# equinor/gordo-components

Hardware: NVIDIA B200
Metric: anomaly windows/sec (64-tag feedforward_hourglass AE, 1k machines x 10k rows per GPU, fused predict+score) (higher is better)
Workload: dtype tf32x3

## Files before the change

gordo_components_b200/csrc/ffae_infer_tc.cu:

```cuda
#include <cuda.h>
#include <atomic>
#include <cstdlib>
#include <cuda_bf16.h>
#include <cuda_fp16.h>
#include "gb_common.cuh"

namespace {

constexpr int TILE = 128;
#ifndef GB_TC_NSLOT
#define GB_TC_NSLOT 2
#endif
#ifndef GB_TC_YPREF
#define GB_TC_YPREF 2
#endif
#ifndef GB_TC_YPREF_LAYER
#define GB_TC_YPREF_LAYER 4
#endif
#ifndef GB_TC_STATIC
#define GB_TC_STATIC 1
#endif
constexpr int NSLOT = GB_TC_NSLOT;
static_assert(NSLOT == 2 || NSLOT == 3, "two or three tile slots");
#ifndef GB_TC_DEDICATED
#define GB_TC_DEDICATED 0
#endif
constexpr int MAIN_WARPS = 8, LAYER_GROUPS = GB_TC_DEDICATED ? NSLOT : 1, OUT0 = MAIN_WARPS * LAYER_GROUPS, OUT_WARPS = 8, EPI_WARPS = OUT0 + OUT_WARPS;
constexpr int NTHREADS = 32 * (EPI_WARPS + NSLOT);
constexpr int MAXL = 8;
constexpr int BOX_BYTES = TILE * 128;
constexpr int OBOX_BYTES = 32 * 128;
constexpr int W = 64;

constexpr uint32_t COL_D = 0, COL_A1 = 64, COL_A2 = 96, COL_ALB = GB_TC_DEDICATED ? 128 : 64, COL_ABF = GB_TC_DEDICATED ? 160 : 96,
                   SLOT_COLS = GB_TC_DEDICATED ? 192 : 128, COL_DX = NSLOT * SLOT_COLS, TMEM_COLS = 512;
static_assert(COL_DX + (GB_TC_DEDICATED ? NSLOT : NSLOT - 1) * 64 <= TMEM_COLS, "tile slots + spare accumulators exceed the 512 TMEM columns");

struct TcArgs {
  int T;
  int n_layers, last_layer;
  int K[MAXL], N[MAXL], Np[MAXL], n8[MAXL], k8[MAXL], k16[MAXL], act[MAXL];
  int whi_ofs[MAXL], wlo_ofs[MAXL], bias_ofs[MAXL];
  int whb_ofs;
  int pofs[MAXL];
  int w_bytes;
  int param_bytes, bulk_params;
  int vec_ofs, xbox_ofs, stage_ofs, pair_ofs, bar_ofs;
  int n_jobs, tiles_per_job, flags;
  long pstride;
  const float* params;
  const gb_job* jobs;
  const float *y, *scale, *feat_thr, *agg_thr;
  float *o_model, *o_ts, *o_tu, *o_conf, *o_tots, *o_totu, *o_totconf;
  unsigned int* work_ctr;
  long long* trace;
  int trace_cap, trace_from, trace_head;
};

enum { FLAG_NO_STORES = 2 };
constexpr int DEFAULT_NE = 0;

constexpr int TRACE_SLOTS = NSLOT == 2 ? 256 : 32;
__device__ __forceinline__ void trace_ev(const TcArgs& a, unsigned long long* ring, int& cnt, int code, int tile, int layer, int slot) {
  if (a.trace == nullptr || blockIdx.x != 0 || cnt >= TRACE_SLOTS || (tile < a.trace_from && tile >= a.trace_head)) return;
  ring[cnt++] = ((unsigned long long)clock64() << 24) | ((unsigned long long)(tile & 0xfff) << 12) | ((layer & 0xf) << 8) | ((slot & 0xf) << 4) | (code & 0xf);
}

__device__ __forceinline__ uint32_t smem_u32(const void* p) { return (uint32_t)__cvta_generic_to_shared(p); }

__device__ __forceinline__ void mbar_init(uint32_t bar, uint32_t count) {
  asm volatile("mbarrier.init.shared::cta.b64 [%0], %1;" ::"r"(bar), "r"(count));
}
__device__ __forceinline__ void mbar_arrive(uint32_t bar) {
  asm volatile("mbarrier.arrive.shared::cta.b64 _, [%0];" ::"r"(bar) : "memory");
}
__device__ __forceinline__ void mbar_expect_tx(uint32_t bar, uint32_t bytes) {
  asm volatile("mbarrier.arrive.expect_tx.shared::cta.b64 _, [%0], %1;" ::"r"(bar), "r"(bytes) : "memory");
}
__device__ __forceinline__ void mbar_wait(uint32_t bar, uint32_t parity) {
  asm volatile(
      "{\n\t"
      ".reg .pred p;\n\t"
      "WAIT_%=:\n\t"
      "mbarrier.try_wait.parity.shared::cta.b64 p, [%0], %1, %2;\n\t"
      "@p bra DONE_%=;\n\t"
      "bra WAIT_%=;\n\t"
      "DONE_%=:\n\t"
      "}" ::"r"(bar), "r"(parity), "r"(0x989680u)
      : "memory");
}
__device__ __forceinline__ void named_bar_sync(int id, int count) { asm volatile("bar.sync %0, %1;" ::"r"(id), "r"(count) : "memory"); }
__device__ __forceinline__ void fence_proxy_async() { asm volatile("fence.proxy.async.shared::cta;" ::: "memory"); }
__device__ __forceinline__ void tc_fence_before() { asm volatile("tcgen05.fence::before_thread_sync;" ::: "memory"); }
__device__ __forceinline__ void tc_fence_after() { asm volatile("tcgen05.fence::after_thread_sync;" ::: "memory"); }

__device__ __forceinline__ void tma_load_2d(uint32_t dst, const CUtensorMap* map, int c0, int c1, uint32_t bar) {
  asm volatile("cp.async.bulk.tensor.2d.shared::cluster.global.mbarrier::complete_tx::bytes [%0], [%1, {%2, %3}], [%4];" ::"r"(dst),
               "l"(map), "r"(c0), "r"(c1), "r"(bar)
               : "memory");
}

__device__ __forceinline__ void mma_bf16_ts(uint32_t d, uint32_t a, uint64_t bdesc, uint32_t idesc, uint32_t accumulate) {
  asm volatile(
      "{\n\t"
      ".reg .pred p;\n\t"
      "setp.ne.b32 p, %4, 0;\n\t"
      "tcgen05.mma.cta_group::1.kind::f16 [%0], [%1], %2, %3, p;\n\t"
      "}" ::"r"(d), "r"(a), "l"(bdesc), "r"(idesc), "r"(accumulate)
      : "memory");
}
__device__ __forceinline__ void mma_tf32_ss(uint32_t d, uint64_t adesc, uint64_t bdesc, uint32_t idesc, uint32_t accumulate) {
  asm volatile(
      "{\n\t"
      ".reg .pred p;\n\t"
      "setp.ne.b32 p, %4, 0;\n\t"
// ... 147 lines not shown
      v[i + j] = (NE > 0 && ((i + j) % (NE > 0 ? NE : 1)) == 0) ? tanh_from_scaled_fma(t[j]) : tanh_from_scaled(t[j]);
  }
  store_a_fp16<NC>(slot_lane, col0, v);
}
template <int C1, int C2, int NE>
__device__ __forceinline__ void hidden_epilogue_pair(uint32_t slot_lane, int c0, const float* bias_all) {
  hidden_epilogue<C1, NE>(slot_lane, c0, bias_all + c0);
  if (C2 > 0) hidden_epilogue<(C2 > 0 ? C2 : 4), NE>(slot_lane, c0 + C1, bias_all + c0 + C1);
}

__device__ __forceinline__ bool elect_one() {
  uint32_t pred;
  asm volatile("{\n\t.reg .pred P;\n\telect.sync _|P, 0xffffffff;\n\tselp.b32 %0, 1, 0, P;\n\t}" : "=r"(pred));
  return pred != 0;
}

template <int V> struct IC {};
constexpr int HG_L = 7;
constexpr int HG_DIMS[HG_L + 1] = {64, 53, 43, 32, 32, 43, 53, 64};
constexpr int hg_ru(int v, int m) { return (v + m - 1) / m * m; }
template <int l> struct HGL {
  static constexpr int K = HG_DIMS[l], N = HG_DIMS[l + 1];
  static constexpr int Np = hg_ru(N, 16), n8 = hg_ru(N, 8), k8 = hg_ru(K, 8) / 8, k16 = hg_ru(K, 16) / 16;
  static constexpr int whi_bytes = l == 0 ? k8 * 8 * Np * 4 : k16 * 16 * Np * 2, wlo_bytes = k16 * 16 * Np * 2, whb_bytes = l == 0 ? k16 * 16 * Np * 2 : 0;
  static constexpr int whi_ofs = HGL<l - 1>::end_ofs, wlo_ofs = whi_ofs + whi_bytes, whb_ofs = wlo_ofs + wlo_bytes, end_ofs = whb_ofs + whb_bytes;
};
template <> struct HGL<-1> { static constexpr int end_ofs = 0; };
template <int l> constexpr int HG_BIAS_OFS = HGL<HG_L - 1>::end_ofs + 64 * 4 * l;

struct LayerP { int K, N, Np, n8, k8, k16, whi_ofs, wlo_ofs, bias_ofs; };
template <int V> __device__ __forceinline__ LayerP layer_of(const TcArgs&, IC<V>) {
  return LayerP{HGL<V>::K, HGL<V>::N, HGL<V>::Np, HGL<V>::n8, HGL<V>::k8, HGL<V>::k16, HGL<V>::whi_ofs, HGL<V>::wlo_ofs, HG_BIAS_OFS<V>};
}
__device__ __forceinline__ LayerP layer_of(const TcArgs& a, int l) {
  return LayerP{a.K[l], a.N[l], a.Np[l], a.n8[l], a.k8[l], a.k16[l], a.whi_ofs[l], a.wlo_ofs[l], a.bias_ofs[l]};
}
template <int V> __device__ __forceinline__ constexpr int layer_index(IC<V>) { return V; }
__device__ __forceinline__ int layer_index(int l) { return l; }
template <bool STATIC, bool HIDDEN_ONLY, class F>
__device__ __forceinline__ void for_layers(int n, F&& f) {
  if constexpr (STATIC) {
    f(IC<0>{}); f(IC<1>{}); f(IC<2>{}); f(IC<3>{}); f(IC<4>{}); f(IC<5>{});
    if constexpr (!HIDDEN_ONLY) f(IC<6>{});
  } else {
    for (int l = 0; l < n; ++l) f(l);
  }
}

template <int NE, bool FULL, bool STATIC>
__global__ void __launch_bounds__(NTHREADS, 1)
ffae_tc_kernel(const __grid_constant__ TcArgs a, const __grid_constant__ CUtensorMap map_x) {
  extern __shared__ __align__(1024) uint8_t smem[];
  __shared__ uint32_t s_tmem_base;
  __shared__ unsigned long long s_trace[4][TRACE_SLOTS];
  int trace_cnt = 0;

  const int tid = threadIdx.x, lane = tid & 31;
  if (a.trace != nullptr && tid == 0) {
    unsigned long long ns;
    asm volatile("mov.u64 %0, %globaltimer;" : "=l"(ns));
    a.trace[8 + 4 * TRACE_SLOTS + 2 * blockIdx.x] = (long long)ns;
    if (blockIdx.x == 0) {
      a.trace[4 + 4 * TRACE_SLOTS + 0] = clock64();
      a.trace[4 + 4 * TRACE_SLOTS + 2] = (long long)ns;
    }
  }
  const int warp = __shfl_sync(0xffffffffu, tid >> 5, 0);
  const bool is_ctrl = warp >= EPI_WARPS, is_out = !is_ctrl && warp >= OUT0;
  unsigned long long* ring = s_trace[is_ctrl ? (warp == EPI_WARPS ? 1 : 0) : (is_out ? (warp == EPI_WARPS - 1 ? 2 : 3) : 0)];
  const int q = warp & 3, h = (warp >> 2) & 1;
  const int row = q * 32 + lane;
  const uint32_t sbase = smem_u32(smem);
  const uint32_t bars = sbase + a.bar_ofs;
  const uint32_t BX = 0, BA = 24, BD = 48, BF = 72, BE = 96, BW = 120, BA0 = 128;
  const bool has_y = a.y != nullptr;
  const int TP = FULL ? W : a.T;
  const int L = STATIC ? HG_L : a.last_layer + 1;

  if (tid == 0) {
    for (int s = 0; s < NSLOT; ++s) {
      mbar_init(bars + BX + 8 * s, 1);
      mbar_init(bars + BA + 8 * s, MAIN_WARPS);
      mbar_init(bars + BA0 + 8 * s, MAIN_WARPS);
      mbar_init(bars + BD + 8 * s, 1);
      mbar_init(bars + BF + 8 * s, 1);
      mbar_init(bars + BE + 8 * s, OUT_WARPS);
    }
    mbar_init(bars + BW, 1);
    asm volatile("fence.mbarrier_init.release.cluster;" ::: "memory");
  }
  if (warp == EPI_WARPS) {
    asm volatile("tcgen05.alloc.cta_group::1.sync.aligned.shared::cta.b32 [%0], %1;" ::"r"(smem_u32(&s_tmem_base)), "n"(TMEM_COLS) : "memory");
    asm volatile("tcgen05.relinquish_alloc_permit.cta_group::1.sync.aligned;" ::: "memory");
  }
  tc_fence_before();
  __syncthreads();
  tc_fence_after();
  const uint32_t tmem = __shfl_sync(0xffffffffu, s_tmem_base, 0);
  const uint32_t lane_base = tmem + ((uint32_t)(q * 32) << 16);

  uint32_t ph_x = 0, ph_d = 0, ph_f = 0;
  uint32_t ph_a = 0, ph_a0 = 0, ph_e = 0, ph_w = 0;
  int cur_slot = -1;
  __shared__ int s_item[4];
  __shared__ int s_range[2];
  if (tid == 0) s_range[0] = s_range[1] = 0;

  while (true) {
    if (tid == 0) {
      const int tpj = a.tiles_per_job, g_total = a.n_jobs * tpj;
      int g = s_range[0], g_end = s_range[1];
      if (g >= g_end) {
        const int seen = (int)*reinterpret_cast<volatile unsigned int*>(a.work_ctr);
        const int left = g_total - seen, per_cta = left / (int)gridDim.x;
        int size = per_cta * 2 >= 3 * tpj ? tpj : (per_cta >= tpj / 3 ? (tpj + 2) / 3 : (tpj + 5) / 6);
        if (size < 1) size = 1;
        if (seen % tpj != 0 && size > tpj - seen % tpj) size = tpj - seen % tpj;
        g = (int)atomicAdd(a.work_ctr, (unsigned int)size);
        g_end = g + size < g_total ? g + size : g_total;
      }
      if (g >= g_total) {
        s_item[0] = -1;
      } else {
        const int job_id = g / tpj, tile_begin = g - job_id * tpj;
        const int tile_end = min(tpj, tile_begin + (g_end - g));
        s_item[0] = job_id; s_item[1] = tile_begin; s_item[2] = tile_end;
        g += tile_end - tile_begin;
      }
      s_range[0] = g; s_range[1] = g_end;
    }
    __syncthreads();
    const int job_id = s_item[0], tile_begin = s_item[1], tile_end = s_item[2];
    if (job_id < 0) break;
    const gb_job job = a.jobs[job_id];
    const int row_begin = tile_begin * TILE;
    if (row_begin >= job.n_rows) {
      __syncthreads();
      continue;
    }
    const int row_end = min(job.n_rows, tile_end * TILE);
    const int n_tiles = (row_end - row_begin + TILE - 1) / TILE;

    if (tid == 0) trace_ev(a, ring, trace_cnt, 13, 0xfff, 0, 0);
    if (job.slot != cur_slot) {
      cur_slot = job.slot;
      const float* P = a.params + (long)job.slot * a.pstride;
      float* scratch = reinterpret_cast<float*>(smem + a.xbox_ofs);
      if (a.bulk_params) {
        if (tid == 0) {
          mbar_expect_tx(bars + BW, (uint32_t)a.param_bytes);
          asm volatile("cp.async.bulk.shared::cluster.global.mbarrier::complete_tx::bytes [%0], [%1], %2, [%3];" ::"r"(smem_u32(scratch)), "l"(P),
                       "r"((uint32_t)a.param_bytes), "r"(bars + BW)
                       : "memory");
        }
      } else {
        for (int i = tid; i < a.param_bytes / 4; i += NTHREADS) scratch[i] = __ldg(P + i);
      }
      const float v_scale = (tid < TP && a.scale) ? __ldg(a.scale + (long)job.slot * TP + tid) : 0.f;
      const float v_thr = (tid < TP && a.feat_thr) ? __ldg(a.feat_thr + (long)job.slot * TP + tid) : 1.f;
      for (int i = tid; i < a.w_bytes / 16; i += NTHREADS) reinterpret_cast<uint4*>(smem)[i] = make_uint4(0, 0, 0, 0);
      __syncthreads();
      if (a.bulk_params) {
        mbar_wait(bars + BW, ph_w);
        ph_w ^= 1;
      }
      for (int l = 0; l < L; ++l) {
        const int K = a.K[l], N = a.N[l], Np = a.Np[l], KN = K * N;
        const float* Ws = scratch + a.pofs[l];
        float* whi = reinterpret_cast<float*>(smem + a.whi_ofs[l]);
        __nv_bfloat16* wlo = reinterpret_cast<__nv_bfloat16*>(smem + a.wlo_ofs[l]);
        __nv_bfloat16* whb = reinterpret_cast<__nv_bfloat16*>(smem + a.whb_ofs);
        for (int k = warp; k < K; k += NTHREADS / 32) {
          const float w0 = lane < N ? Ws[k * N + lane] : 0.f, w1v = lane + 32 < N ? Ws[k * N + lane + 32] : 0.f;
#pragma unroll
          for (int u = 0; u < 2; ++u) {
            const int n = lane + 32 * u;
            const float w = u ? w1v : w0;
            if (n < N) {
              if (l == 0) {
                const float hi = __uint_as_float((__float_as_uint(w) + 0x1000u) & 0xffffe000u);
                whi[((k >> 2) * Np + n) * 4 + (k & 3)] = hi;
                wlo[((k >> 3) * Np + n) * 8 + (k & 7)] = __float2bfloat16_rn(w - hi);
                whb[((k >> 3) * Np + n) * 8 + (k & 7)] = __float2bfloat16_rn(hi);
              } else {
                const __half w1 = __float2half_rn(w);
                reinterpret_cast<__half*>(whi)[((k >> 3) * Np + n) * 8 + (k & 7)] = w1;
                reinterpret_cast<__half*>(wlo)[((k >> 3) * Np + n) * 8 + (k & 7)] = __float2half_rn(w - __half2float(w1));
              }
            }
          }
        }
        float* bl = reinterpret_cast<float*>(smem + a.bias_ofs[l]);
        const float bscale = (l + 1 < L) ? TANH_ARG_SCALE : 1.0f;
        for (int n = tid; n < N; n += NTHREADS) bl[n] = Ws[KN + n] * bscale;
      }
      float* vec = reinterpret_cast<float*>(smem + a.vec_ofs);
      if (tid < W) {
        vec[tid] = v_scale;
        vec[W + tid] = (a.feat_thr && tid < TP) ? 1.0f / v_thr : 0.f;
      }
      fence_proxy_async();
    }
    __syncthreads();
    if (tid == 0) trace_ev(a, ring, trace_cnt, 14, 0xfff, 0, 0);

    auto split_wait_x = [&](int tt) {
      const int s = tt % NSLOT;
      mbar_wait(bars + BX + 8 * s, (ph_x >> s) & 1u);
      ph_x ^= 1u << s;
    };
    auto split_piece = [&](int tt, int piece) {
      const int s = tt % NSLOT;
      const uint32_t xbox = sbase + a.xbox_ofs + (2 * s + h) * BOX_BYTES + (uint32_t)row * 128u;
      float v[8];
#pragma unroll
      for (int c = 0; c < 2; ++c) {
        const uint32_t addr = xbox + ((uint32_t)((piece * 2 + c) ^ (row & 7)) << 4);
        asm volatile("ld.shared.v4.f32 {%0,%1,%2,%3}, [%4];" : "=f"(v[4 * c]), "=f"(v[4 * c + 1]), "=f"(v[4 * c + 2]), "=f"(v[4 * c + 3]) : "r"(addr));
      }
      store_a_operands<8>(lane_base + s * SLOT_COLS, h * 32 + piece * 8, v);
    };
    auto split_done = [&](int tt) {
      const int s = tt % NSLOT;
      tmem_wait_st();
      tc_fence_before();
      __syncwarp();
      if (lane == 0) mbar_arrive(bars + (GB_TC_DEDICATED ? BA0 : BA) + 8 * s);
      if (lane == 0 && (warp == OUT0 || (GB_TC_DEDICATED && warp == 0))) trace_ev(a, ring, trace_cnt, 3, tt, 0, s);
    };
    auto split_x = [&](int tt) {
      split_wait_x(tt);
#pragma unroll
      for (int piece = 0; piece < 4; ++piece) split_piece(tt, piece);
      split_done(tt);
    };
    if (is_ctrl) {
      const int s = warp - EPI_WARPS;
      const long xrow0 = job.x_row + row_begin;
      const uint32_t bar_x = bars + BX + 8 * s, bar_a = bars + BA + 8 * s, bar_d = bars + BD + 8 * s, bar_f = bars + BF + 8 * s,
                     bar_e = bars + BE + 8 * s;
      const uint32_t xdst = sbase + a.xbox_ofs + s * 2 * BOX_BYTES;
      const uint32_t tb = tmem + s * SLOT_COLS;
      const uint32_t whb_ofs = STATIC ? HGL<0>::whb_ofs : a.whb_ofs;
      auto prefetch_y = [&](int t) {
        if (has_y) {
          const int nrows = min(TILE, row_end - (row_begin + t * TILE));
          asm volatile("cp.async.bulk.prefetch.L2.global [%0], %1;" ::"l"(a.y + (xrow0 + (long)t * TILE) * TP), "r"((uint32_t)(nrows * TP * 4)) : "memory");
        }
      };
      auto fetch_tile = [&](int t) {
        mbar_expect_tx(bar_x, 2 * BOX_BYTES);
        tma_load_2d(xdst, &map_x, 0, (int)(xrow0 + (long)t * TILE), bar_x);
        tma_load_2d(xdst + BOX_BYTES, &map_x, 32, (int)(xrow0 + (long)t * TILE), bar_x);
        if (GB_TC_YPREF == 1) prefetch_y(t);
      };
      if (s < n_tiles && elect_one()) fetch_tile(s);
      __syncwarp();
      for (int t = s; t < n_tiles; t += NSLOT) {
        for_layers<STATIC, false>(L, [&](auto lc) {
          const int l = layer_index(lc);
          const LayerP P = layer_of(a, lc);
          const int Np = P.Np, k8 = P.k8, k16 = P.k16;
          const uint32_t id32 = make_idesc(2, Np), id16 = make_idesc(l == 0 ? 1 : 0, Np);
          const uint32_t lbo = (uint32_t)Np * 16u;
          const uint32_t dstep = 2u * (uint32_t)Np;
          const uint64_t dhi = make_bdesc(sbase + P.whi_ofs, lbo, 128), dlo = make_bdesc(sbase + P.wlo_ofs, lbo, 128), dhb = make_bdesc(sbase + whb_ofs, lbo, 128);
          if (GB_TC_DEDICATED && l == 0) {
            mbar_wait(bars + BA0 + 8 * s, ph_a0);
            ph_a0 ^= 1;
          } else {
            mbar_wait(bar_a, ph_a);
            ph_a ^= 1;
          }
          if (t >= NSLOT && l == ((s == 0 && !GB_TC_DEDICATED) ? 0 : L - 1)) {
            mbar_wait(bar_e, ph_e);
            ph_e ^= 1;
          }
          const uint32_t dcol = (l == L - 1 && (GB_TC_DEDICATED || s >= 1)) ? tmem + COL_DX + (uint32_t)(GB_TC_DEDICATED ? s : s - 1) * 64u : tb + COL_D;
          tc_fence_after();
          if (elect_one()) {
            if (s == 0) trace_ev(a, ring, trace_cnt, 1, t, l, s);
            if (GB_TC_YPREF == 2 && l == (L > GB_TC_YPREF_LAYER ? GB_TC_YPREF_LAYER : 0)) prefetch_y(t);
            if (l == 1 && t + NSLOT < n_tiles) fetch_tile(t + NSLOT);
            if (l == 0) {
#pragma unroll
              for (int ks = 0; ks < 8; ++ks)
                if (ks < k8) mma_tf32_ss(dcol, make_adesc_sw128(xdst + (ks >> 2) * BOX_BYTES) + (uint64_t)((ks & 3) * 2), dhi + (uint64_t)(ks * dstep), id32, ks > 0);
#pragma unroll
              for (int ks = 0; ks < 4; ++ks)
                if (ks < k16) mma_bf16_ts(dcol, tb + COL_ALB + ks * 8, dhb + (uint64_t)(ks * dstep), id16, 1);
#pragma unroll
              for (int ks = 0; ks < 4; ++ks)
                if (ks < k16) mma_bf16_ts(dcol, tb + COL_ABF + ks * 8, dlo + (uint64_t)(ks * dstep), id16, 1);
            } else {
#pragma unroll
              for (int ks = 0; ks < 4; ++ks)
                if (ks < k16) mma_bf16_ts(dcol, tb + COL_A2 + ks * 8, dhi + (uint64_t)(ks * dstep), id16, ks > 0);
#pragma unroll
              for (int ks = 0; ks < 4; ++ks)
                if (ks < k16) mma_bf16_ts(dcol, tb + COL_A1 + ks * 8, dlo + (uint64_t)(ks * dstep), id16, 1);
#pragma unroll
              for (int ks = 0; ks < 4; ++ks)
                if (ks < k16) mma_bf16_ts(dcol, tb + COL_A1 + ks * 8, dhi + (uint64_t)(ks * dstep), id16, 1);
            }
            if (l + 1 < L) {
              mma_commit(bar_d);
            } else {
              mma_commit(bar_f);
            }
            if (s == 0) trace_ev(a, ring, trace_cnt, 2, t, l, s);
          }
          __syncwarp();
        });
      }
      if (s < n_tiles) ph_e ^= 1;
    } else if (!is_out) {
      const int grp = GB_TC_DEDICATED ? warp / MAIN_WARPS : 0;
      auto serve = [&](int s, int t, auto lc) {
        const int l = layer_index(lc);
        const LayerP P = layer_of(a, lc);
        const int half = P.n8 >> 1;
        const float* bl = reinterpret_cast<const float*>(smem + P.bias_ofs);
        tc_fence_after();
        if (tid == 0) trace_ev(a, ring, trace_cnt, 5, t, l, s);
        const uint32_t sl = lane_base + s * SLOT_COLS;
        const int c0 = h * half;
        switch (half) {
          case 32: hidden_epilogue_pair<16, 16, NE>(sl, c0, bl); break;
          case 28: hidden_epilogue_pair<16, 12, NE>(sl, c0, bl); break;
          case 24: hidden_epilogue_pair<12, 12, NE>(sl, c0, bl); break;
          case 20: hidden_epilogue_pair<12, 8, NE>(sl, c0, bl); break;
          case 16: hidden_epilogue_pair<8, 8, NE>(sl, c0, bl); break;
          case 12: hidden_epilogue_pair<8, 4, NE>(sl, c0, bl); break;
          case 8: hidden_epilogue_pair<4, 4, NE>(sl, c0, bl); break;
          default: hidden_epilogue_pair<4, 0, NE>(sl, c0, bl); break;
        }
        if (h == 1 && P.n8 < P.Np) {
          const uint32_t z[4] = {0u, 0u, 0u, 0u};
          tmem_st4(sl + COL_A1 + (P.n8 >> 1), z);
          tmem_st4(sl + COL_A2 + (P.n8 >> 1), z);
        }
        tmem_wait_st();
        tc_fence_before();
        __syncwarp();
        if (lane == 0) mbar_arrive(bars + BA + 8 * s);
        if (tid == 0) trace_ev(a, ring, trace_cnt, 6, t, l, s);
      };
      if (GB_TC_DEDICATED) {
        const int H = L - 1;
        if (grp < n_tiles) split_x(grp);
        for (int t = grp; t < n_tiles; t += NSLOT) {
          const bool more = t + NSLOT < n_tiles;
          for_layers<STATIC, true>(H, [&](auto lc) {
            const int l = layer_index(lc);
            mbar_wait(bars + BD + 8 * grp, (ph_d >> grp) & 1u);
            ph_d ^= 1u << grp;
            if (l == 0 && t >= NSLOT) {
              mbar_wait(bars + BF + 8 * grp, (ph_f >> grp) & 1u);
              ph_f ^= 1u << grp;
            }
            serve(grp, t, lc);
            if (more) {
              const int first = H > 1 ? 1 : 0;
              const int lo = H > 1 ? 4 * (l - 1) / (H - 1) : 0, hi = H > 1 ? 4 * l / (H - 1) : 4;
              if (l == first) split_wait_x(t + NSLOT);
              if (l >= first)
                for (int piece = lo; piece < hi; ++piece) split_piece(t + NSLOT, piece);
              if (l == H - 1) split_done(t + NSLOT);
            }
          });
        }
        if (grp < n_tiles) {
          mbar_wait(bars + BF + 8 * grp, (ph_f >> grp) & 1u);
          ph_f ^= 1u << grp;
        }
      } else {
        for (int t0 = 0; t0 < n_tiles; t0 += NSLOT) {
          for_layers<STATIC, true>(L - 1, [&](auto lc) {
#pragma unroll
            for (int s = 0; s < NSLOT; ++s) {
              if (t0 + s >= n_tiles) continue;
              if (tid == 0) trace_ev(a, ring, trace_cnt, 4, t0 + s, layer_index(lc), s);
              mbar_wait(bars + BD + 8 * s, (ph_d >> s) & 1u);
              ph_d ^= 1u << s;
              serve(s, t0 + s, lc);
            }
          });
        }
      }
    } else {
      const float* vec = reinterpret_cast<const float*>(smem + a.vec_ofs);
      const uint32_t stage = sbase + a.stage_ofs + (warp - OUT0) * OBOX_BYTES;
      float* pair = reinterpret_cast<float*>(smem + a.pair_ofs);
      const int tr = lane >> 3, tc = lane & 7;
      const float4 sc4 = *reinterpret_cast<const float4*>(vec + h * 32 + tc * 4);
      const float4 rt4 = *reinterpret_cast<const float4*>(vec + W + h * 32 + tc * 4);
      const float4 b4 = *reinterpret_cast<const float4*>(reinterpret_cast<const float*>(smem + (STATIC ? HG_BIAS_OFS<HG_L - 1> : a.bias_ofs[L - 1])) + h * 32 + tc * 4);
      const float inv_w = 1.0f / (float)TP;
      const bool in_cols = FULL || h * 32 + tc * 4 < TP;
      const bool totals = has_y && (a.o_tots || a.o_totu || a.o_totconf);

      auto park = [&](int s, int t) {
        float acc[32];
        const uint32_t sl = lane_base + ((GB_TC_DEDICATED || s >= 1) ? COL_DX + (uint32_t)(GB_TC_DEDICATED ? s : s - 1) * 64u : COL_D) + h * 32;
#pragma unroll
        for (int c = 0; c < 4; ++c) tmem_ld8_nowait(sl + 8 * c, acc + 8 * c);
#pragma unroll
        for (int c = 0; c < 4; ++c) tmem_wait_ld8(acc + 8 * c);
        tc_fence_before();
        __syncwarp();
        if (lane == 0) mbar_arrive(bars + BE + 8 * s);
        if (lane == 0 && (warp == OUT0 || warp == EPI_WARPS - 1)) trace_ev(a, ring, trace_cnt, 10, t, L - 1, s);
#pragma unroll
        for (int c = 0; c < 8; ++c) {
          const uint32_t addr = stage + (uint32_t)lane * 128u + ((uint32_t)(c ^ (lane & 7)) << 4);
          asm volatile("st.shared.v4.f32 [%0], {%1,%2,%3,%4};" ::"r"(addr), "f"(acc[4 * c]), "f"(acc[4 * c + 1]), "f"(acc[4 * c + 2]), "f"(acc[4 * c + 3]) : "memory");
        }
        __syncwarp();
      };
      auto y_row = [&](int t, int i) -> float4 {
        const int trow = row_begin + t * TILE;
        const int r = min(q * 32 + i * 4 + tr, min(TILE, row_end - trow) - 1);
        return in_cols ? __ldg(reinterpret_cast<const float4*>(a.y + (job.x_row + trow + r) * (long)TP + h * 32) + tc) : make_float4(0.f, 0.f, 0.f, 0.f);
      };
      constexpr int YW = 3;
      float4 yt[GB_TC_DEDICATED ? YW : 8];
      auto emit = [&](int t) {
        const int trow = row_begin + t * TILE;
        const int nrows = min(TILE, row_end - trow);
        const long grow0 = job.out_row + trow;
        const int wrow0 = q * 32;
        float ss[8], su[8];
#pragma unroll
        for (int i = 0; i < 8; ++i) {
          const int r = i * 4 + tr;
          float4 yh, yv = yt[GB_TC_DEDICATED ? i % YW : i];
          if (GB_TC_DEDICATED && has_y && i + YW < 8) yt[i % YW] = y_row(t, i + YW);
          const uint32_t addr = stage + (uint32_t)r * 128u + ((uint32_t)(tc ^ (r & 7)) << 4);
          asm volatile("ld.shared.v4.f32 {%0,%1,%2,%3}, [%4];" : "=f"(yh.x), "=f"(yh.y), "=f"(yh.z), "=f"(yh.w) : "r"(addr));
          if (!in_cols) yv = make_float4(0.f, 0.f, 0.f, 0.f);
          yh.x += b4.x; yh.y += b4.y; yh.z += b4.z; yh.w += b4.w;
          if (!in_cols) yh = make_float4(0.f, 0.f, 0.f, 0.f);
          const bool live = wrow0 + r < nrows && in_cols && !(a.flags & FLAG_NO_STORES);
          const long g = (grow0 + wrow0 + r) * (long)TP + h * 32 + tc * 4;
          if (live) __stcs(reinterpret_cast<float4*>(a.o_model + g), yh);
          ss[i] = 0.f; su[i] = 0.f;
          if (has_y) {
            float4 d, e;
            d.x = fabsf(yh.x - yv.x); d.y = fabsf(yh.y - yv.y); d.z = fabsf(yh.z - yv.z); d.w = fabsf(yh.w - yv.w);
            su[i] = d.x * d.x + d.y * d.y + d.z * d.z + d.w * d.w;
            if (live && a.o_tu) __stcs(reinterpret_cast<float4*>(a.o_tu + g), d);
            e.x = d.x * sc4.x; e.y = d.y * sc4.y; e.z = d.z * sc4.z; e.w = d.w * sc4.w;
            ss[i] = e.x * e.x + e.y * e.y + e.z * e.z + e.w * e.w;
            if (live && a.o_ts) __stcs(reinterpret_cast<float4*>(a.o_ts + g), e);
            if (live && a.o_conf) __stcs(reinterpret_cast<float4*>(a.o_conf + g), make_float4(d.x * rt4.x, d.y * rt4.y, d.z * rt4.z, d.w * rt4.w));
          }
        }
        __syncwarp();
        if (lane == 0 && (warp == OUT0 || warp == EPI_WARPS - 1)) trace_ev(a, ring, trace_cnt, 12, t, L - 1, t % NSLOT);
        if (totals) {
#pragma unroll
          for (int i = 0; i < 8; ++i) {
#pragma unroll
            for (int o = 1; o < 8; o <<= 1) {
              ss[i] += __shfl_xor_sync(0xffffffffu, ss[i], o);
              su[i] += __shfl_xor_sync(0xffffffffu, su[i], o);
            }
            if (tc == 0) {
              pair[h * 2 * TILE + wrow0 + i * 4 + tr] = ss[i];
              pair[h * 2 * TILE + TILE + wrow0 + i * 4 + tr] = su[i];
            }
          }
          named_bar_sync(1 + q, 64);
          if (h == 0 && row < nrows) {
            const float ts_ = (pair[row] + pair[2 * TILE + row]) * inv_w, tu_ = (pair[TILE + row] + pair[3 * TILE + row]) * inv_w;
            if (a.o_tots) a.o_tots[grow0 + row] = ts_;
            if (a.o_totu) a.o_totu[grow0 + row] = tu_;
            if (a.o_totconf) a.o_totconf[grow0 + row] = ts_ / __ldg(a.agg_thr + job.slot);
          }
          named_bar_sync(1 + q, 64);
        }
        if (lane == 0 && (warp == OUT0 || warp == EPI_WARPS - 1)) trace_ev(a, ring, trace_cnt, 9, t, L - 1, t % NSLOT);
      };

      auto load_y = [&](int t) {
#pragma unroll
        for (int i = 0; i < (GB_TC_DEDICATED ? YW : 8); ++i) yt[i] = y_row(t, i);
      };
      auto wait_f = [&](int s, int t) {
        mbar_wait(bars + BF + 8 * s, (ph_f >> s) & 1u);
        ph_f ^= 1u << s;
        tc_fence_after();
        if (lane == 0 && (warp == OUT0 || warp == EPI_WARPS - 1)) trace_ev(a, ring, trace_cnt, 8, t, L - 1, s);
      };

      if (GB_TC_DEDICATED) {
        for (int t = 0; t < n_tiles; ++t) {
          const int s = t % NSLOT;
          if (has_y) load_y(t);
          wait_f(s, t);
          park(s, t);
          emit(t);
        }
      } else {
      split_x(0);
      if (n_tiles > 1) split_x(1);
      if (NSLOT > 2 && n_tiles > 2) split_x(2);

      for (int t0 = 0; t0 < n_tiles; t0 += NSLOT) {
        const int n_in = min(NSLOT, n_tiles - t0);
        if (has_y) load_y(t0);
        if (lane == 0 && (warp == OUT0 || warp == EPI_WARPS - 1)) trace_ev(a, ring, trace_cnt, 7, t0, L - 1, 0);
        wait_f(0, t0);
        park(0, t0);
        if (t0 + NSLOT < n_tiles) split_x(t0 + NSLOT);
        if (n_in > 1) {
          wait_f(1, t0 + 1);
          if (t0 + NSLOT + 1 < n_tiles) split_x(t0 + NSLOT + 1);
        }
        if (n_in > 2) {
          wait_f(2, t0 + 2);
          if (t0 + NSLOT + 2 < n_tiles) split_x(t0 + NSLOT + 2);
        }
        emit(t0);
        if (n_in > 1) {
          if (has_y) load_y(t0 + 1);
          park(1, t0 + 1);
          emit(t0 + 1);
        }
        if (n_in > 2) {
          if (has_y) load_y(t0 + 2);
          park(2, t0 + 2);
          emit(t0 + 2);
        }
      }
      }
    }
    fence_proxy_async();
    __syncthreads();
  }

  if (a.trace != nullptr && tid == 0) {
    unsigned long long ns;
    asm volatile("mov.u64 %0, %globaltimer;" : "=l"(ns));
    a.trace[8 + 4 * TRACE_SLOTS + 2 * blockIdx.x + 1] = (long long)ns;
    if (blockIdx.x == 0) {
      a.trace[4 + 4 * TRACE_SLOTS + 1] = clock64();
      a.trace[4 + 4 * TRACE_SLOTS + 3] = (long long)ns;
    }
  }
  if (a.trace != nullptr && blockIdx.x == 0 && lane == 0 && (warp == 0 || warp == OUT0 || warp == EPI_WARPS - 1 || warp == EPI_WARPS)) {
    const int role = is_ctrl ? 1 : (is_out ? (warp == EPI_WARPS - 1 ? 2 : 3) : 0);
    a.trace[role] = trace_cnt;
    for (int i = 0; i < trace_cnt; ++i) a.trace[4 + role * TRACE_SLOTS + i] = (long long)ring[i];
  }
  tc_fence_before();
  __syncthreads();
  if (warp == EPI_WARPS) asm volatile("tcgen05.dealloc.cta_group::1.sync.aligned.b32 %0, %1;" ::"r"(tmem), "n"(TMEM_COLS) : "memory");
}

typedef CUresult (*EncodeTiledFn)(CUtensorMap*, CUtensorMapDataType, cuuint32_t, void*, const cuuint64_t*, const cuuint64_t*,
                                  const cuuint32_t*, const cuuint32_t*, CUtensorMapInterleave, CUtensorMapSwizzle,
                                  CUtensorMapL2promotion, CUtensorMapFloatOOBfill);

EncodeTiledFn get_encode_fn() {
  static EncodeTiledFn fn = nullptr;
  if (fn) return fn;
  void* p = nullptr;
  cudaDriverEntryPointQueryResult qres;
  if (cudaGetDriverEntryPoint("cuTensorMapEncodeTiled", &p, cudaEnableDefault, &qres) != cudaSuccess || qres != cudaDriverEntryPointSuccess) return nullptr;
  fn = reinterpret_cast<EncodeTiledFn>(p);
  return fn;
}

int make_map(CUtensorMap* map, const void* base, int64_t rows, int box_rows, int T) {
  EncodeTiledFn fn = get_encode_fn();
  GB_REQUIRE(fn != nullptr, GB_E_CUDA, "cuTensorMapEncodeTiled is not available from the driver");
  cuuint64_t dims[2] = {(cuuint64_t)T, (cuuint64_t)(rows > 0 ? rows : 1)};
  cuuint64_t strides[1] = {(cuuint64_t)T * sizeof(float)};
  cuuint32_t box[2] = {32, (cuuint32_t)box_rows};
  cuuint32_t estr[2] = {1, 1};
  CUresult r = fn(map, CU_TENSOR_MAP_DATA_TYPE_FLOAT32, 2, const_cast<void*>(base), dims, strides, box, estr, CU_TENSOR_MAP_INTERLEAVE_NONE,
                  CU_TENSOR_MAP_SWIZZLE_128B, CU_TENSOR_MAP_L2_PROMOTION_L2_128B, CU_TENSOR_MAP_FLOAT_OOB_FILL_NONE);
  GB_REQUIRE(r == CUDA_SUCCESS, GB_E_CUDA, "cuTensorMapEncodeTiled failed with CUresult %d", (int)r);
  return GB_OK;
}

constexpr int WORK_CTRS = 1024;
// ... 28 lines not shown
      gb::set_error("tcgen05 variant is specialised for tanh hidden layers and a linear output (the factory defaults)");
      return GB_E_SHAPE;
    }
  return GB_OK;
}

extern "C" int gb_ffae_infer_score_tc(const gb_ffnet* net, const float* params, const gb_job* jobs, int32_t n_jobs, int32_t max_rows,
                                      int64_t n_x_rows, int64_t n_out_rows, const float* x, const float* y, const float* scale,
                                      const float* feat_thr, const float* agg_thr, float* out_model, float* out_tag_scaled,
                                      float* out_tag_unscaled, float* out_total_scaled, float* out_total_unscaled, float* out_conf,
                                      float* out_total_conf, int32_t flags, void* stream) {
  int rc = gb_ffae_tc_supported(net);
  if (rc != GB_OK) return rc;
  GB_REQUIRE(n_x_rows > 0 && n_out_rows > 0, GB_E_ARG, "the tcgen05 variant needs the row counts of x and of the outputs");
  TcArgs a{};
  const int L = net->n_layers;
  a.n_layers = L;
  a.T = net->dims[0];
  const int dbg_last = (flags >> 8) & 0xff;
  a.last_layer = (dbg_last > 0 && dbg_last <= L) ? dbg_last - 1 : L - 1;
  a.flags = flags & 0xff;
  int ofs = 0, pofs = 0;
  for (int l = 0; l < L; ++l) {
    a.K[l] = net->dims[l];
    a.N[l] = net->dims[l + 1];
    a.Np[l] = gb::round_up(a.N[l], 16);
    a.n8[l] = gb::round_up(a.N[l], 8);
    a.k8[l] = gb::round_up(a.K[l], 8) / 8;
    a.k16[l] = gb::round_up(a.K[l], 16) / 16;
    a.act[l] = net->act[l];
    a.pofs[l] = pofs;
    pofs += a.K[l] * a.N[l] + a.N[l];
    a.whi_ofs[l] = ofs;
    ofs += l == 0 ? a.k8[l] * 8 * a.Np[l] * 4 : a.k16[l] * 16 * a.Np[l] * 2;
    a.wlo_ofs[l] = ofs;
    ofs += a.k16[l] * 16 * a.Np[l] * 2;
    if (l == 0) {
      a.whb_ofs = ofs;
      ofs += a.k16[l] * 16 * a.Np[l] * 2;
    }
  }
  for (int l = 0; l < L; ++l) {
    a.bias_ofs[l] = ofs;
    ofs += 64 * 4;
  }
  a.w_bytes = gb::round_up(ofs, 16);
  ofs = a.w_bytes;
  a.vec_ofs = ofs; ofs += 2 * W * 4;
  a.pair_ofs = ofs; ofs += 4 * TILE * 4;
  a.bar_ofs = ofs; ofs += 192;
  ofs = gb::round_up(ofs, 1024);
  a.xbox_ofs = ofs; ofs += 2 * NSLOT * BOX_BYTES;
  a.stage_ofs = ofs; ofs += OUT_WARPS * OBOX_BYTES;
  const size_t smem = (size_t)ofs;
  GB_REQUIRE(smem + 4 * TRACE_SLOTS * 8 + 64 <= 227 * 1024, GB_E_SMEM, "architecture needs %zu bytes of shared memory in the tcgen05 variant", smem);

  int dev = 0, sms = 148;
  GB_CUDA_CHECK(cudaGetDevice(&dev));
  GB_CUDA_CHECK(cudaDeviceGetAttribute(&sms, cudaDevAttrMultiProcessorCount, dev));
  const int tiles_per_job = (max_rows + TILE - 1) / TILE;
  a.tiles_per_job = tiles_per_job;
  a.n_jobs = n_jobs;
  a.pstride = (long)gb_ffnet_param_stride(net);
  a.param_bytes = (int)(gb_ffnet_param_stride(net) * sizeof(float));
  GB_REQUIRE(a.param_bytes <= 2 * NSLOT * BOX_BYTES + OUT_WARPS * OBOX_BYTES, GB_E_SMEM, "parameter vector of %d bytes exceeds the staging scratch", a.param_bytes);
  a.bulk_params = (reinterpret_cast<uintptr_t>(params) % 16 == 0) ? 1 : 0;
  a.params = params; a.jobs = jobs; a.y = y; a.scale = scale; a.feat_thr = feat_thr; a.agg_thr = agg_thr;
  a.o_model = out_model; a.o_ts = out_tag_scaled; a.o_tu = out_tag_unscaled; a.o_conf = out_conf;
  a.o_tots = out_total_scaled; a.o_totu = out_total_unscaled; a.o_totconf = out_total_conf;
  a.trace = g_trace; a.trace_cap = g_trace_cap;
  if (const char* e = getenv("GB_TC_TRACE_FROM")) a.trace_from = atoi(e);
  if (const char* e = getenv("GB_TC_TRACE_HEAD")) a.trace_head = atoi(e);

  CUtensorMap mx;
  if ((rc = make_map(&mx, x, n_x_rows, TILE, a.T)) != GB_OK) return rc;

  const long g_total = (long)n_jobs * tiles_per_job;
  const int grid = (int)(g_total < sms ? g_total : sms);
  {
    static std::atomic<unsigned> next_ctr{0};
    void* base = nullptr;
    GB_CUDA_CHECK(cudaGetSymbolAddress(&base, g_work_ctr));
    GB_REQUIRE(g_total < (1L << 31), GB_E_ARG, "%ld tiles in one launch: split the fleet", g_total);
    a.work_ctr = static_cast<unsigned int*>(base) + (next_ctr.fetch_add(1) % WORK_CTRS);
    GB_CUDA_CHECK(cudaMemsetAsync(a.work_ctr, 0, sizeof(unsigned int), (cudaStream_t)stream));
  }
  auto launch = [&](auto kern) -> int {
    GB_CUDA_CHECK(cudaFuncSetAttribute(kern, cudaFuncAttributeMaxDynamicSharedMemorySize, (int)smem));
    kern<<<grid, NTHREADS, smem, (cudaStream_t)stream>>>(a, mx);
    return GB_OK;
  };
  bool hg = GB_TC_STATIC && L == HG_L && a.last_layer == L - 1 && a.whb_ofs == HGL<0>::whb_ofs;
  for (int l = 0; hg && l <= L; ++l) hg = net->dims[l] == HG_DIMS[l];
  {
    const int want_whi[HG_L] = {HGL<0>::whi_ofs, HGL<1>::whi_ofs, HGL<2>::whi_ofs, HGL<3>::whi_ofs, HGL<4>::whi_ofs, HGL<5>::whi_ofs, HGL<6>::whi_ofs};
    const int want_wlo[HG_L] = {HGL<0>::wlo_ofs, HGL<1>::wlo_ofs, HGL<2>::wlo_ofs, HGL<3>::wlo_ofs, HGL<4>::wlo_ofs, HGL<5>::wlo_ofs, HGL<6>::wlo_ofs};
    const int want_bias[HG_L] = {HG_BIAS_OFS<0>, HG_BIAS_OFS<1>, HG_BIAS_OFS<2>, HG_BIAS_OFS<3>, HG_BIAS_OFS<4>, HG_BIAS_OFS<5>, HG_BIAS_OFS<6>};
    for (int l = 0; hg && l < L; ++l) hg = a.whi_ofs[l] == want_whi[l] && a.wlo_ofs[l] == want_wlo[l] && a.bias_ofs[l] == want_bias[l];
  }
  rc = hg ? launch(ffae_tc_kernel<DEFAULT_NE, true, true>)
          : (a.T == W ? launch(ffae_tc_kernel<DEFAULT_NE, true, false>) : launch(ffae_tc_kernel<DEFAULT_NE, false, false>));
  if (rc != GB_OK) return rc;
  GB_CUDA_CHECK(cudaGetLastError());
  return GB_OK;
}
```

Baseline: 3.242 billion.

## Stage target rows via bulk async copy into shared memory; drop dedicated-group mode

Replaces per-thread __ldg reads of the target y rows in the output warps with a single cp.async.bulk of the whole tile into a new shared buffer, signalled by an mbarrier and double-checked by a consumer-release barrier so the next tile's fetch starts once all output warps have read. It also removes the compile-time dedicated layer-group variant and moves the trace ring into dynamic shared memory. The intent is to take global-load latency for y off the epilogue's critical path. The cost is extra shared memory (TILE*T*4 bytes), a single y buffer that serialises fetch against consumption, and a new 16-byte alignment requirement on y.

```diff
diff --git a/gordo_components_b200/csrc/ffae_infer_tc.cu b/gordo_components_b200/csrc/ffae_infer_tc.cu
--- a/gordo_components_b200/csrc/ffae_infer_tc.cu
+++ b/gordo_components_b200/csrc/ffae_infer_tc.cu
@@ -22,19 +22,15 @@
 #endif
 constexpr int NSLOT = GB_TC_NSLOT;
 static_assert(NSLOT == 2 || NSLOT == 3, "two or three tile slots");
-#ifndef GB_TC_DEDICATED
-#define GB_TC_DEDICATED 0
-#endif
-constexpr int MAIN_WARPS = 8, LAYER_GROUPS = GB_TC_DEDICATED ? NSLOT : 1, OUT0 = MAIN_WARPS * LAYER_GROUPS, OUT_WARPS = 8, EPI_WARPS = OUT0 + OUT_WARPS;
+constexpr int MAIN_WARPS = 8, OUT0 = MAIN_WARPS, OUT_WARPS = 8, EPI_WARPS = OUT0 + OUT_WARPS;
 constexpr int NTHREADS = 32 * (EPI_WARPS + NSLOT);
 constexpr int MAXL = 8;
 constexpr int BOX_BYTES = TILE * 128;
 constexpr int OBOX_BYTES = 32 * 128;
 constexpr int W = 64;
 
-constexpr uint32_t COL_D = 0, COL_A1 = 64, COL_A2 = 96, COL_ALB = GB_TC_DEDICATED ? 128 : 64, COL_ABF = GB_TC_DEDICATED ? 160 : 96,
-                   SLOT_COLS = GB_TC_DEDICATED ? 192 : 128, COL_DX = NSLOT * SLOT_COLS, TMEM_COLS = 512;
-static_assert(COL_DX + (GB_TC_DEDICATED ? NSLOT : NSLOT - 1) * 64 <= TMEM_COLS, "tile slots + spare accumulators exceed the 512 TMEM columns");
+constexpr uint32_t COL_D = 0, COL_A1 = 64, COL_A2 = 96, COL_ALB = 64, COL_ABF = 96, SLOT_COLS = 128, COL_DX = NSLOT * SLOT_COLS, TMEM_COLS = 512;
+static_assert(COL_DX + (NSLOT - 1) * 64 <= TMEM_COLS, "tile slots + spare accumulators exceed the 512 TMEM columns");
 
 struct TcArgs {
   int T;
@@ -45,7 +41,8 @@
   int pofs[MAXL];
   int w_bytes;
   int param_bytes, bulk_params;
-  int vec_ofs, xbox_ofs, stage_ofs, pair_ofs, bar_ofs;
+  int vec_ofs, xbox_ofs, stage_ofs, ybuf_ofs, pair_ofs, bar_ofs;
+  int trace_ofs;
   int n_jobs, tiles_per_job, flags;
   long pstride;
   const float* params;
@@ -60,7 +57,7 @@
 enum { FLAG_NO_STORES = 2 };
 constexpr int DEFAULT_NE = 0;
 
-constexpr int TRACE_SLOTS = NSLOT == 2 ? 256 : 32;
+constexpr int TRACE_SLOTS = NSLOT == 2 ? 128 : 32;
 __device__ __forceinline__ void trace_ev(const TcArgs& a, unsigned long long* ring, int& cnt, int code, int tile, int layer, int slot) {
   if (a.trace == nullptr || blockIdx.x != 0 || cnt >= TRACE_SLOTS || (tile < a.trace_from && tile >= a.trace_head)) return;
   ring[cnt++] = ((unsigned long long)clock64() << 24) | ((unsigned long long)(tile & 0xfff) << 12) | ((layer & 0xf) << 8) | ((slot & 0xf) << 4) | (code & 0xf);
@@ -314,7 +311,6 @@
 ffae_tc_kernel(const __grid_constant__ TcArgs a, const __grid_constant__ CUtensorMap map_x) {
   extern __shared__ __align__(1024) uint8_t smem[];
   __shared__ uint32_t s_tmem_base;
-  __shared__ unsigned long long s_trace[4][TRACE_SLOTS];
   int trace_cnt = 0;
 
   const int tid = threadIdx.x, lane = tid & 31;
@@ -329,12 +325,13 @@
   }
   const int warp = __shfl_sync(0xffffffffu, tid >> 5, 0);
   const bool is_ctrl = warp >= EPI_WARPS, is_out = !is_ctrl && warp >= OUT0;
-  unsigned long long* ring = s_trace[is_ctrl ? (warp == EPI_WARPS ? 1 : 0) : (is_out ? (warp == EPI_WARPS - 1 ? 2 : 3) : 0)];
+  unsigned long long* ring = reinterpret_cast<unsigned long long*>(smem + a.trace_ofs) +
+                             TRACE_SLOTS * (is_ctrl ? (warp == EPI_WARPS ? 1 : 0) : (is_out ? (warp == EPI_WARPS - 1 ? 2 : 3) : 0));
   const int q = warp & 3, h = (warp >> 2) & 1;
   const int row = q * 32 + lane;
   const uint32_t sbase = smem_u32(smem);
   const uint32_t bars = sbase + a.bar_ofs;
-  const uint32_t BX = 0, BA = 24, BD = 48, BF = 72, BE = 96, BW = 120, BA0 = 128;
+  const uint32_t BX = 0, BA = 24, BD = 48, BF = 72, BE = 96, BW = 120, BY = 128, BYF = 136;
   const bool has_y = a.y != nullptr;
   const int TP = FULL ? W : a.T;
   const int L = STATIC ? HG_L : a.last_layer + 1;
@@ -343,12 +340,13 @@
     for (int s = 0; s < NSLOT; ++s) {
       mbar_init(bars + BX + 8 * s, 1);
       mbar_init(bars + BA + 8 * s, MAIN_WARPS);
-      mbar_init(bars + BA0 + 8 * s, MAIN_WARPS);
       mbar_init(bars + BD + 8 * s, 1);
       mbar_init(bars + BF + 8 * s, 1);
       mbar_init(bars + BE + 8 * s, OUT_WARPS);
     }
     mbar_init(bars + BW, 1);
+    mbar_init(bars + BY, 1);
+    mbar_init(bars + BYF, OUT_WARPS);
     asm volatile("fence.mbarrier_init.release.cluster;" ::: "memory");
   }
   if (warp == EPI_WARPS) {
@@ -362,7 +360,8 @@
   const uint32_t lane_base = tmem + ((uint32_t)(q * 32) << 16);
 
   uint32_t ph_x = 0, ph_d = 0, ph_f = 0;
-  uint32_t ph_a = 0, ph_a0 = 0, ph_e = 0, ph_w = 0;
+  constexpr int PH_Y = 4;
+  uint32_t ph_a = 0, ph_e = 0, ph_w = 0;
   int cur_slot = -1;
   __shared__ int s_item[4];
   __shared__ int s_range[2];
@@ -466,35 +465,26 @@
     __syncthreads();
     if (tid == 0) trace_ev(a, ring, trace_cnt, 14, 0xfff, 0, 0);
 
-    auto split_wait_x = [&](int tt) {
+    auto split_x = [&](int tt) {
       const int s = tt % NSLOT;
       mbar_wait(bars + BX + 8 * s, (ph_x >> s) & 1u);
       ph_x ^= 1u << s;
-    };
-    auto split_piece = [&](int tt, int piece) {
-      const int s = tt % NSLOT;
       const uint32_t xbox = sbase + a.xbox_ofs + (2 * s + h) * BOX_BYTES + (uint32_t)row * 128u;
-      float v[8];
-#pragma unroll
-      for (int c = 0; c < 2; ++c) {
-        const uint32_t addr = xbox + ((uint32_t)((piece * 2 + c) ^ (row & 7)) << 4);
-        asm volatile("ld.shared.v4.f32 {%0,%1,%2,%3}, [%4];" : "=f"(v[4 * c]), "=f"(v[4 * c + 1]), "=f"(v[4 * c + 2]), "=f"(v[4 * c + 3]) : "r"(addr));
-      }
-      store_a_operands<8>(lane_base + s * SLOT_COLS, h * 32 + piece * 8, v);
-    };
-    auto split_done = [&](int tt) {
-      const int s = tt % NSLOT;
+#pragma unroll
+      for (int piece = 0; piece < 4; ++piece) {
+        float v[8];
+#pragma unroll
+        for (int c = 0; c < 2; ++c) {
+          const uint32_t addr = xbox + ((uint32_t)((piece * 2 + c) ^ (row & 7)) << 4);
+          asm volatile("ld.shared.v4.f32 {%0,%1,%2,%3}, [%4];" : "=f"(v[4 * c]), "=f"(v[4 * c + 1]), "=f"(v[4 * c + 2]), "=f"(v[4 * c + 3]) : "r"(addr));
+        }
+        store_a_operands<8>(lane_base + s * SLOT_COLS, h * 32 + piece * 8, v);
+      }
       tmem_wait_st();
       tc_fence_before();
       __syncwarp();
-      if (lane == 0) mbar_arrive(bars + (GB_TC_DEDICATED ? BA0 : BA) + 8 * s);
-      if (lane == 0 && (warp == OUT0 || (GB_TC_DEDICATED && warp == 0))) trace_ev(a, ring, trace_cnt, 3, tt, 0, s);
-    };
-    auto split_x = [&](int tt) {
-      split_wait_x(tt);
-#pragma unroll
-      for (int piece = 0; piece < 4; ++piece) split_piece(tt, piece);
-      split_done(tt);
+      if (lane == 0) mbar_arrive(bars + BA + 8 * s);
+      if (lane == 0 && warp == OUT0) trace_ev(a, ring, trace_cnt, 3, tt, 0, s);
     };
     if (is_ctrl) {
       const int s = warp - EPI_WARPS;
@@ -527,18 +517,13 @@
           const uint32_t lbo = (uint32_t)Np * 16u;
           const uint32_t dstep = 2u * (uint32_t)Np;
           const uint64_t dhi = make_bdesc(sbase + P.whi_ofs, lbo, 128), dlo = make_bdesc(sbase + P.wlo_ofs, lbo, 128), dhb = make_bdesc(sbase + whb_ofs, lbo, 128);
-          if (GB_TC_DEDICATED && l == 0) {
-            mbar_wait(bars + BA0 + 8 * s, ph_a0);
-            ph_a0 ^= 1;
-          } else {
-            mbar_wait(bar_a, ph_a);
-            ph_a ^= 1;
-          }
-          if (t >= NSLOT && l == ((s == 0 && !GB_TC_DEDICATED) ? 0 : L - 1)) {
+          mbar_wait(bar_a, ph_a);
+          ph_a ^= 1;
+          if (t >= NSLOT && l == (s == 0 ? 0 : L - 1)) {
             mbar_wait(bar_e, ph_e);
             ph_e ^= 1;
           }
-          const uint32_t dcol = (l == L - 1 && (GB_TC_DEDICATED || s >= 1)) ? tmem + COL_DX + (uint32_t)(GB_TC_DEDICATED ? s : s - 1) * 64u : tb + COL_D;
+          const uint32_t dcol = (l == L - 1 && s >= 1) ? tmem + COL_DX + (uint32_t)(s - 1) * 64u : tb + COL_D;
           tc_fence_after();
           if (elect_one()) {
             if (s == 0) trace_ev(a, ring, trace_cnt, 1, t, l, s);
@@ -577,7 +562,6 @@
       }
       if (s < n_tiles) ph_e ^= 1;
     } else if (!is_out) {
-      const int grp = GB_TC_DEDICATED ? warp / MAIN_WARPS : 0;
       auto serve = [&](int s, int t, auto lc) {
         const int l = layer_index(lc);
         const LayerP P = layer_of(a, lc);
@@ -608,47 +592,17 @@
         if (lane == 0) mbar_arrive(bars + BA + 8 * s);
         if (tid == 0) trace_ev(a, ring, trace_cnt, 6, t, l, s);
       };
-      if (GB_TC_DEDICATED) {
-        const int H = L - 1;
-        if (grp < n_tiles) split_x(grp);
-        for (int t = grp; t < n_tiles; t += NSLOT) {
-          const bool more = t + NSLOT < n_tiles;
-          for_layers<STATIC, true>(H, [&](auto lc) {
-            const int l = layer_index(lc);
-            mbar_wait(bars + BD + 8 * grp, (ph_d >> grp) & 1u);
-            ph_d ^= 1u << grp;
-            if (l == 0 && t >= NSLOT) {
-              mbar_wait(bars + BF + 8 * grp, (ph_f >> grp) & 1u);
-              ph_f ^= 1u << grp;
-            }
-            serve(grp, t, lc);
-            if (more) {
-              const int first = H > 1 ? 1 : 0;
-              const int lo = H > 1 ? 4 * (l - 1) / (H - 1) : 0, hi = H > 1 ? 4 * l / (H - 1) : 4;
-              if (l == first) split_wait_x(t + NSLOT);
-              if (l >= first)
-                for (int piece = lo; piece < hi; ++piece) split_piece(t + NSLOT, piece);
-              if (l == H - 1) split_done(t + NSLOT);
-            }
-          });
-        }
-        if (grp < n_tiles) {
-          mbar_wait(bars + BF + 8 * grp, (ph_f >> grp) & 1u);
-          ph_f ^= 1u << grp;
-        }
-      } else {
-        for (int t0 = 0; t0 < n_tiles; t0 += NSLOT) {
-          for_layers<STATIC, true>(L - 1, [&](auto lc) {
-#pragma unroll
-            for (int s = 0; s < NSLOT; ++s) {
-              if (t0 + s >= n_tiles) continue;
-              if (tid == 0) trace_ev(a, ring, trace_cnt, 4, t0 + s, layer_index(lc), s);
-              mbar_wait(bars + BD + 8 * s, (ph_d >> s) & 1u);
-              ph_d ^= 1u << s;
-              serve(s, t0 + s, lc);
-            }
-          });
-        }
+      for (int t0 = 0; t0 < n_tiles; t0 += NSLOT) {
+        for_layers<STATIC, true>(L - 1, [&](auto lc) {
+#pragma unroll
+          for (int s = 0; s < NSLOT; ++s) {
+            if (t0 + s >= n_tiles) continue;
+            if (tid == 0) trace_ev(a, ring, trace_cnt, 4, t0 + s, layer_index(lc), s);
+            mbar_wait(bars + BD + 8 * s, (ph_d >> s) & 1u);
+            ph_d ^= 1u << s;
+            serve(s, t0 + s, lc);
+          }
+        });
       }
     } else {
       const float* vec = reinterpret_cast<const float*>(smem + a.vec_ofs);
@@ -664,7 +618,7 @@
 
       auto park = [&](int s, int t) {
         float acc[32];
-        const uint32_t sl = lane_base + ((GB_TC_DEDICATED || s >= 1) ? COL_DX + (uint32_t)(GB_TC_DEDICATED ? s : s - 1) * 64u : COL_D) + h * 32;
+        const uint32_t sl = lane_base + (s >= 1 ? COL_DX + (uint32_t)(s - 1) * 64u : COL_D) + h * 32;
 #pragma unroll
         for (int c = 0; c < 4; ++c) tmem_ld8_nowait(sl + 8 * c, acc + 8 * c);
 #pragma unroll
@@ -680,13 +634,7 @@
         }
         __syncwarp();
       };
-      auto y_row = [&](int t, int i) -> float4 {
-        const int trow = row_begin + t * TILE;
-        const int r = min(q * 32 + i * 4 + tr, min(TILE, row_end - trow) - 1);
-        return in_cols ? __ldg(reinterpret_cast<const float4*>(a.y + (job.x_row + trow + r) * (long)TP + h * 32) + tc) : make_float4(0.f, 0.f, 0.f, 0.f);
-      };
-      constexpr int YW = 3;
-      float4 yt[GB_TC_DEDICATED ? YW : 8];
+      float4 yt[8];
       auto emit = [&](int t) {
         const int trow = row_begin + t * TILE;
         const int nrows = min(TILE, row_end - trow);
@@ -696,8 +644,7 @@
 #pragma unroll
         for (int i = 0; i < 8; ++i) {
           const int r = i * 4 + tr;
-          float4 yh, yv = yt[GB_TC_DEDICATED ? i % YW : i];
-          if (GB_TC_DEDICATED && has_y && i + YW < 8) yt[i % YW] = y_row(t, i + YW);
+          float4 yh, yv = yt[i];
           const uint32_t addr = stage + (uint32_t)r * 128u + ((uint32_t)(tc ^ (r & 7)) << 4);
           asm volatile("ld.shared.v4.f32 {%0,%1,%2,%3}, [%4];" : "=f"(yh.x), "=f"(yh.y), "=f"(yh.z), "=f"(yh.w) : "r"(addr));
           if (!in_cols) yv = make_float4(0.f, 0.f, 0.f, 0.f);
@@ -745,9 +692,37 @@
         if (lane == 0 && (warp == OUT0 || warp == EPI_WARPS - 1)) trace_ev(a, ring, trace_cnt, 9, t, L - 1, t % NSLOT);
       };
 
+      auto fetch_y = [&](int t) {
+        const int trow = row_begin + t * TILE;
+        const uint32_t bytes = (uint32_t)(min(TILE, row_end - trow) * TP * 4);
+        mbar_expect_tx(bars + BY, bytes);
+        asm volatile("cp.async.bulk.shared::cluster.global.mbarrier::complete_tx::bytes [%0], [%1], %2, [%3];" ::"r"(sbase + a.ybuf_ofs),
+                     "l"(a.y + (job.x_row + trow) * (long)TP), "r"(bytes), "r"(bars + BY)
+                     : "memory");
+      };
       auto load_y = [&](int t) {
-#pragma unroll
-        for (int i = 0; i < (GB_TC_DEDICATED ? YW : 8); ++i) yt[i] = y_row(t, i);
+        const int nrows = min(TILE, row_end - (row_begin + t * TILE));
+        mbar_wait(bars + BY, (ph_x >> PH_Y) & 1u);
+        ph_x ^= 1u << PH_Y;
+#pragma unroll
+        for (int i = 0; i < 8; ++i) {
+          const int r = min(q * 32 + i * 4 + tr, nrows - 1);
+          const uint32_t addr = sbase + a.ybuf_ofs + (uint32_t)(r * TP + h * 32 + tc * 4) * 4u;
+          if (in_cols) {
+            asm volatile("ld.shared.v4.f32 {%0,%1,%2,%3}, [%4];" : "=f"(yt[i].x), "=f"(yt[i].y), "=f"(yt[i].z), "=f"(yt[i].w) : "r"(addr) : "memory");
+          } else {
+            yt[i] = make_float4(0.f, 0.f, 0.f, 0.f);
+          }
+        }
+        __syncwarp();
+        if (lane == 0) mbar_arrive(bars + BYF);
+        if (warp == OUT0) {
+          if (t + 1 < n_tiles && elect_one()) {
+            mbar_wait(bars + BYF, ((ph_x >> PH_Y) & 1u) ^ 1u);
+            fetch_y(t + 1);
+          }
+          __syncwarp();
+        }
       };
       auto wait_f = [&](int s, int t) {
         mbar_wait(bars + BF + 8 * s, (ph_f >> s) & 1u);
@@ -756,15 +731,10 @@
         if (lane == 0 && (warp == OUT0 || warp == EPI_WARPS - 1)) trace_ev(a, ring, trace_cnt, 8, t, L - 1, s);
       };
 
-      if (GB_TC_DEDICATED) {
-        for (int t = 0; t < n_tiles; ++t) {
-          const int s = t % NSLOT;
-          if (has_y) load_y(t);
-          wait_f(s, t);
-          park(s, t);
-          emit(t);
-        }
-      } else {
+      if (has_y && warp == OUT0) {
+        if (elect_one()) fetch_y(0);
+        __syncwarp();
+      }
       split_x(0);
       if (n_tiles > 1) split_x(1);
       if (NSLOT > 2 && n_tiles > 2) split_x(2);
@@ -795,7 +765,6 @@
           park(2, t0 + 2);
           emit(t0 + 2);
         }
-      }
       }
     }
     fence_proxy_async();
@@ -930,8 +899,11 @@
   ofs = gb::round_up(ofs, 1024);
   a.xbox_ofs = ofs; ofs += 2 * NSLOT * BOX_BYTES;
   a.stage_ofs = ofs; ofs += OUT_WARPS * OBOX_BYTES;
+  a.ybuf_ofs = ofs; ofs += TILE * a.T * 4;
+  a.trace_ofs = ofs;
+  if (g_trace != nullptr) ofs += 4 * TRACE_SLOTS * 8;
   const size_t smem = (size_t)ofs;
-  GB_REQUIRE(smem + 4 * TRACE_SLOTS * 8 + 64 <= 227 * 1024, GB_E_SMEM, "architecture needs %zu bytes of shared memory in the tcgen05 variant", smem);
+  GB_REQUIRE(smem + 1024 <= 227 * 1024, GB_E_SMEM, "architecture needs %zu bytes of shared memory in the tcgen05 variant", smem);
 
   int dev = 0, sms = 148;
   GB_CUDA_CHECK(cudaGetDevice(&dev));
@@ -943,6 +915,7 @@
   a.param_bytes = (int)(gb_ffnet_param_stride(net) * sizeof(float));
   GB_REQUIRE(a.param_bytes <= 2 * NSLOT * BOX_BYTES + OUT_WARPS * OBOX_BYTES, GB_E_SMEM, "parameter vector of %d bytes exceeds the staging scratch", a.param_bytes);
   a.bulk_params = (reinterpret_cast<uintptr_t>(params) % 16 == 0) ? 1 : 0;
+  GB_REQUIRE(reinterpret_cast<uintptr_t>(y) % 16 == 0, GB_E_ARG, "the tcgen05 variant needs y 16-byte aligned (its rows are fetched by bulk copy)");
   a.params = params; a.jobs = jobs; a.y = y; a.scale = scale; a.feat_thr = feat_thr; a.agg_thr = agg_thr;
   a.o_model = out_model; a.o_ts = out_tag_scaled; a.o_tu = out_tag_unscaled; a.o_conf = out_conf;
   a.o_tots = out_total_scaled; a.o_totu = out_total_unscaled; a.o_totconf = out_total_conf;
```

After: 3.264 billion, median of 6. No clear change (+0.7%).
